# lucaspk512/vrdone

Hardware: AMD Instinct MI355X
Metric: subject-object pairs/sec forward (2048 pairs x 256 frames x 512-d) (higher is better)
Workload: dtype f16x3: f32 products as 3 scaled-f16 MFMA products (~22-bit), f32 accumulate; reference-grade: distance to a float64 run of the reference <= 1.4 x the reference's own float32 error (tests/golden/mask_vrd_f64.npz)

## Files before the change

vrdone_amd/csrc/vrd_gemm_epilogue.h:

```cpp
#pragma once
#include "vrd_common.h"
#include <type_traits>

namespace vrd {

using f32x16 = __attribute__((ext_vector_type(16))) float;
constexpr int STG_PITCH = 64;

typedef float f32x4_t __attribute__((ext_vector_type(4)));
struct acc32q {
    f32x4_t b[2][2];
};
__device__ __forceinline__ void acc_clear(f32x16& a) {
#pragma unroll
    for (int e = 0; e < 16; ++e) a[e] = 0.f;
}
__device__ __forceinline__ void acc_clear(acc32q& a) {
#pragma unroll
    for (int i = 0; i < 2; ++i)
#pragma unroll
        for (int j = 0; j < 2; ++j)
#pragma unroll
            for (int e = 0; e < 4; ++e) a.b[i][j][e] = 0.f;
}
template <typename Fn>
__device__ __forceinline__ void forall32(const f32x16& a, int lane, Fn&& f) {
    const int li = lane & 31, lh = lane >> 5;
#pragma unroll
    for (int e = 0; e < 16; ++e) f((e & 3) + 8 * (e >> 2) + 4 * lh, li, a[e]);
}
template <typename Fn>
__device__ __forceinline__ void forall32(const acc32q& a, int lane, Fn&& f) {
    const int lc = lane & 15, lq = lane >> 4;
#pragma unroll
    for (int bi = 0; bi < 2; ++bi)
#pragma unroll
        for (int bj = 0; bj < 2; ++bj)
#pragma unroll
            for (int j = 0; j < 4; ++j) f(16 * bi + 4 * lq + j, 16 * bj + lc, a.b[bi][bj][j]);
}

__device__ __forceinline__ float epilogue_value(const vrd_gemm_args& p, float v, float mk, float scale, float r1, float rmk,
                                                float r2) {
    if (p.act == VRD_ACT_RELU) v = fmaxf(v, 0.f);
    else if (p.act == VRD_ACT_GELU) v = gelu_erf(v);
    return v * mk * scale + r1 * rmk + r2;
}

struct EpiCols {
    float bias[4], scale[4];
    float alpha;
};
__device__ __forceinline__ float acc_alpha(const vrd_gemm_args& p) {
    if (!(p.split_fmt == VRD_PAIR_F16 && p.w_scale)) return 1.0f;
    const float alpha = uniform_load(p.w_scale);
    return (p.a_scale && p.a_pair_width == 0) ? alpha * F16_ACT_SCALE * uniform_load(p.a_scale + 1) : alpha;
}
__device__ __forceinline__ EpiCols load_epi_cols(const vrd_gemm_args& p, int nw, int lane) {
    EpiCols c;
    c.alpha = acc_alpha(p);
    const int n = nw + (lane & 15) * 4;
#pragma unroll
    for (int j = 0; j < 4; ++j) c.bias[j] = 0.f, c.scale[j] = 1.f;
    if (n + 3 < p.N) {
        if (p.bias) {
            const float4 b = gload4(p.bias + n);
            c.bias[0] = b.x, c.bias[1] = b.y, c.bias[2] = b.z, c.bias[3] = b.w;
        }
        if (p.scale) {
            const float4 b = gload4(p.scale + n);
            c.scale[0] = b.x, c.scale[1] = b.y, c.scale[2] = b.z, c.scale[3] = b.w;
        }
    }
    return c;
}

__device__ __forceinline__ EpiCols load_epi_cols_async(const vrd_gemm_args& p, int nw, int lane) {
    EpiCols c;
    c.alpha = acc_alpha(p);
    const int n = nw + (lane & 15) * 4;
    float4 b = make_float4(0.f, 0.f, 0.f, 0.f), sc = make_float4(1.f, 1.f, 1.f, 1.f);
    if (n + 3 < p.N) {
        if (p.bias) asm volatile("global_load_dwordx4 %0, %1, off" : "=v"(b) : "v"(p.bias + n) : "memory");
        if (p.scale) asm volatile("global_load_dwordx4 %0, %1, off" : "=v"(sc) : "v"(p.scale + n) : "memory");
    }
    c.bias[0] = b.x, c.bias[1] = b.y, c.bias[2] = b.z, c.bias[3] = b.w;
    c.scale[0] = sc.x, c.scale[1] = sc.y, c.scale[2] = sc.z, c.scale[3] = sc.w;
    return c;
}

template <bool ROWIN, int ACT, int SLAB, int ROWS, typename Transposer>
__device__ __forceinline__ void gemm_epilogue_lean_tr(const vrd_gemm_args& p, Transposer&& transpose_into, float* stg, int64_t mw,
                                                      int64_t mw1, int nw, int lane, const EpiCols& cols, unsigned* rflag = nullptr) {
    RangeTrack rt;
    const int64_t hop = mw1 - (mw + 32);
    const int c4 = (lane & 15) * 4, rb0 = lane >> 4;
    const int n = nw + c4;
    const int64_t m_lane = mw + rb0;
    const bool pair = p.c_pair != 0;
    char* const c_lane = reinterpret_cast<char*>(p.C + m_lane * p.ldc) + (pair ? pair_index(n) * 2 : n * 4);
    const float* const r1_lane = (ROWIN && p.res) ? p.res + m_lane * p.ldres + n : nullptr;
    const float* const r2_lane = (ROWIN && p.res2) ? p.res2 + m_lane * p.ldres2 + n : nullptr;
    const unsigned char* const mk_lane = (ROWIN && p.row_mask) ? p.row_mask + m_lane : nullptr;
    const int64_t c_step = p.ldc * 16, r1_step = p.ldres * 4, r2_step = p.ldres2 * 4;
    const int64_t c_hop = hop * p.ldc * 4;
    struct RowIn {
        unsigned char mb[4];
        float4 r1[4], r2[4];
    };
    auto fetch = [&](int pass) {
        RowIn in;
        if (ROWIN) {
            if (p.row_mask) {
#pragma unroll
                for (int j = 0; j < 4; ++j) in.mb[j] = *as_global(mk_lane + pass * 16 + 4 * j + (pass >= 2 ? hop : 0));
            }
            if (p.res) {
#pragma unroll
                for (int j = 0; j < 4; ++j)
                    in.r1[j] = gload4(r1_lane + (pass * 4 + j) * r1_step + (pass >= 2 ? hop * p.ldres : 0));
            }
            if (p.res2) {
#pragma unroll
                for (int j = 0; j < 4; ++j)
                    in.r2[j] = gload4(r2_lane + (pass * 4 + j) * r2_step + (pass >= 2 ? hop * p.ldres2 : 0));
            }
        }
        return in;
    };
    constexpr int NPASS = ROWS / 16;
    RowIn q0 = fetch(0), q1 = fetch(1);
    unsigned rd_addr[4];
    {
        typedef __attribute__((address_space(3))) const float* lds_cf;
#pragma unroll
        for (int j = 0; j < 4; ++j) rd_addr[j] = (unsigned)reinterpret_cast<uintptr_t>((lds_cf)(stg + (rb0 + 4 * j) * STG_PITCH + (c4 ^ (16 * j))));
    }
    transpose_into(stg, SLAB == 64 ? -1 : 0);
#pragma unroll
    for (int pass = 0; pass < NPASS; ++pass) {
        if (SLAB == 32 && pass == 2) transpose_into(stg, 1);
        const RowIn cur = q0;
        q0 = q1;
        if (pass + 2 < NPASS) q1 = fetch(pass + 2);
        float v[4][4];
        float4 tr[4];
        {
            constexpr int PASS_OFF = (SLAB == 64 ? 1 : 0);
            const int poff = (PASS_OFF ? pass : (pass & 1)) * 16 * STG_PITCH * 4;
            asm volatile("ds_read_b128 %0, %4 offset:%8\n\tds_read_b128 %1, %5 offset:%8\n\tds_read_b128 %2, %6 offset:%8\n\tds_read_b128 %3, %7 offset:%8\n\t"
                         "s_waitcnt lgkmcnt(0)"
                         : "=&v"(tr[0]), "=&v"(tr[1]), "=&v"(tr[2]), "=&v"(tr[3])
                         : "v"(rd_addr[0]), "v"(rd_addr[1]), "v"(rd_addr[2]), "v"(rd_addr[3]), "n"(poff)
                         : "memory");
        }
#pragma unroll
        for (int j = 0; j < 4; ++j) {
            const float4 t = tr[j];
            v[j][0] = fmaf(t.x, cols.alpha, cols.bias[0]), v[j][1] = fmaf(t.y, cols.alpha, cols.bias[1]);
            v[j][2] = fmaf(t.z, cols.alpha, cols.bias[2]), v[j][3] = fmaf(t.w, cols.alpha, cols.bias[3]);
        }
        if (ACT == VRD_ACT_GELU) {
#pragma unroll
            for (int j = 0; j < 4; ++j)
#pragma unroll
                for (int c = 0; c < 4; c += 2) {
                    f32x2_t t2;
                    t2.x = v[j][c], t2.y = v[j][c + 1];
                    t2 = gelu_erf2(t2);
                    v[j][c] = t2.x, v[j][c + 1] = t2.y;
                }
        }
        if (ROWIN) {
            float mk[4] = {1.f, 1.f, 1.f, 1.f};
            if (p.row_mask) {
#pragma unroll
                for (int j = 0; j < 4; ++j) mk[j] = (float)cur.mb[j];
            }
            if (p.row_mask || p.scale) {
#pragma unroll
                for (int j = 0; j < 4; ++j)
#pragma unroll
                    for (int c = 0; c < 4; ++c) v[j][c] *= mk[j] * cols.scale[c];
            }
            if (p.res) {
#pragma unroll
                for (int j = 0; j < 4; ++j) {
                    const float rmk = p.res_masked ? mk[j] : 1.f;
                    v[j][0] += cur.r1[j].x * rmk, v[j][1] += cur.r1[j].y * rmk;
                    v[j][2] += cur.r1[j].z * rmk, v[j][3] += cur.r1[j].w * rmk;
                }
            }
            if (p.res2) {
#pragma unroll
                for (int j = 0; j < 4; ++j) {
                    v[j][0] += cur.r2[j].x, v[j][1] += cur.r2[j].y;
                    v[j][2] += cur.r2[j].z, v[j][3] += cur.r2[j].w;
                }
            }
        }
        if (pair) {
            if (p.c_pair == VRD_PAIR_F16) {
#pragma unroll
                for (int j = 0; j < 4; ++j) {
                    char* const rowp = c_lane + (pass * 4 + j) * c_step + (pass >= 2 ? c_hop : 0);
                    f16x4_t h, l;
                    split_n<true>(v[j], h, l, &rt);
                    *as_global(reinterpret_cast<f16x4_t*>(rowp)) = h;
                    *as_global(reinterpret_cast<f16x4_t*>(rowp + 64)) = l;
                }
            } else {
#pragma unroll
                for (int j = 0; j < 4; ++j) {
                    char* const rowp = c_lane + (pass * 4 + j) * c_step + (pass >= 2 ? c_hop : 0);
                    bf16x4_t h, l;
                    split_n<false>(v[j], h, l);
                    *as_global(reinterpret_cast<bf16x4_t*>(rowp)) = h;
                    *as_global(reinterpret_cast<bf16x4_t*>(rowp + 64)) = l;
                }
            }
        } else {
#pragma unroll
            for (int j = 0; j < 4; ++j)
                gstore4(c_lane + (pass * 4 + j) * c_step + (pass >= 2 ? c_hop : 0), make_float4(v[j][0], v[j][1], v[j][2], v[j][3]));
        }
    }
    if (p.c_pair == VRD_PAIR_F16) rt.report(rflag, RANGE_GEMM_OUT);
}

template <bool ROWIN, int ACT, int SLAB = 64>
__device__ __forceinline__ void gemm_epilogue_lean16(const vrd_gemm_args& p, const f32x4_t (&acc)[4][4], float* stg, int64_t mw,
                                                     int64_t mw1, int nw, int lane, const EpiCols& cols, unsigned* rflag = nullptr) {
    const int lc = lane & 15, lq = lane >> 4;
    gemm_epilogue_lean_tr<ROWIN, ACT, SLAB, 64>(
        p,
        [&](float* slab, int half) {
#pragma unroll
            for (int ti = 0; ti < 4; ++ti) {
                if (half >= 0 && (ti >> 1) != half) continue;
                const int r0 = half < 0 ? ti * 16 : (ti & 1) * 16;
#pragma unroll
                for (int tj = 0; tj < 4; ++tj)
#pragma unroll
                    for (int j = 0; j < 4; ++j) slab[(r0 + 4 * lq + j) * STG_PITCH + (tj ^ lq) * 16 + lc] = acc[ti][tj][j];
            }
        },
        stg, mw, mw1, nw, lane, cols, rflag);
}

inline bool gemm_epilogue_lean_ok(const vrd_gemm_args& a) {
    auto al16 = [](const void* q) { return (reinterpret_cast<uintptr_t>(q) & 15u) == 0; };
    return a.M % 64 == 0 && a.N % 64 == 0 && (a.act == VRD_ACT_NONE || a.act == VRD_ACT_GELU) &&
           !(a.act == VRD_ACT_GELU && (a.row_mask || a.scale || a.res || a.res2)) && al16(a.bias) && al16(a.scale);
}

template <bool STAGED, int SLAB_ROWS = 32, typename Acc>
__device__ __forceinline__ void gemm_epilogue(const vrd_gemm_args& p, const Acc (&acc)[2][2], float* smem, int64_t mw,
                                              int nw, int wave, int lane, unsigned* rflag = nullptr, int64_t mw1 = -1) {
    if (mw1 < 0) mw1 = mw + 32;
    auto rowbase = [&](int mi) { return mi ? mw1 : mw; };
    RangeTrack rt;
    constexpr bool SWZ = std::is_same<Acc, acc32q>::value;
    if (STAGED) {
        float* stg = smem + wave * (SLAB_ROWS * STG_PITCH);
        const int c4 = (lane & 15) * 4, rb0 = lane >> 4;
        const int n = nw + c4;
        const bool nfull = n + 3 < p.N;
        const float alpha = acc_alpha(p);
        float bias[4] = {0.f, 0.f, 0.f, 0.f}, scale[4] = {1.f, 1.f, 1.f, 1.f};
        if (nfull && ((reinterpret_cast<uintptr_t>(p.bias) | reinterpret_cast<uintptr_t>(p.scale)) & 15) == 0) {
            if (p.bias) {
                const float4 b = *reinterpret_cast<const float4*>(p.bias + n);
                bias[0] = b.x, bias[1] = b.y, bias[2] = b.z, bias[3] = b.w;
            }
            if (p.scale) {
                const float4 b = *reinterpret_cast<const float4*>(p.scale + n);
                scale[0] = b.x, scale[1] = b.y, scale[2] = b.z, scale[3] = b.w;
            }
        } else {
#pragma unroll
            for (int j = 0; j < 4; ++j)
                if (n + j < p.N) {
                    if (p.bias) bias[j] = p.bias[n + j];
                    if (p.scale) scale[j] = p.scale[n + j];
                }
        }
        const bool row_inputs = p.row_mask || p.res || p.res2;
        const bool ragged = __any(n < p.N && !nfull);
        struct RowIn {
            float mk[4];
            float4 r1[4], r2[4];
        };
        auto fetch = [&](int pass) {
            RowIn in;
#pragma unroll
            for (int j = 0; j < 4; ++j) {
                in.mk[j] = 1.f;
                in.r1[j] = make_float4(0.f, 0.f, 0.f, 0.f);
                in.r2[j] = in.r1[j];
            }
            if (!row_inputs) return in;
            const int64_t mr = rowbase(pass >> 1) + rb0 + (pass & 1) * 16;
            if (!ragged) {
                const int nc = n < p.N ? n : 0;
                unsigned char mb[4];
                int64_t mc[4];
#pragma unroll
                for (int j = 0; j < 4; ++j) mc[j] = (mr + 4 * j < p.M) ? mr + 4 * j : p.M - 1;
                if (p.row_mask) {
#pragma unroll
                    for (int j = 0; j < 4; ++j) mb[j] = p.row_mask[mc[j]];
                }
                if (p.res) {
#pragma unroll
                    for (int j = 0; j < 4; ++j) in.r1[j] = *reinterpret_cast<const float4*>(p.res + mc[j] * p.ldres + nc);
                }
                if (p.res2) {
#pragma unroll
                    for (int j = 0; j < 4; ++j) in.r2[j] = *reinterpret_cast<const float4*>(p.res2 + mc[j] * p.ldres2 + nc);
                }
                if (p.row_mask) {
#pragma unroll
                    for (int j = 0; j < 4; ++j) in.mk[j] = (float)mb[j];
                }
                return in;
            }
#pragma unroll
            for (int j = 0; j < 4; ++j) {
                const int64_t m = mr + 4 * j;
                const bool ok = m < p.M && n < p.N;
                if (p.row_mask && ok) in.mk[j] = (float)p.row_mask[m];
                if (ok && nfull) {
                    if (p.res) in.r1[j] = *reinterpret_cast<const float4*>(p.res + m * p.ldres + n);
                    if (p.res2) in.r2[j] = *reinterpret_cast<const float4*>(p.res2 + m * p.ldres2 + n);
                } else if (ok) {
                    float a1[4] = {0.f, 0.f, 0.f, 0.f}, a2[4] = {0.f, 0.f, 0.f, 0.f};
#pragma unroll
                    for (int c = 0; c < 4; ++c)
                        if (n + c < p.N) {
                            if (p.res) a1[c] = p.res[m * p.ldres + n + c];
                            if (p.res2) a2[c] = p.res2[m * p.ldres2 + n + c];
                        }
                    in.r1[j] = make_float4(a1[0], a1[1], a1[2], a1[3]);
                    in.r2[j] = make_float4(a2[0], a2[1], a2[2], a2[3]);
                }
            }
            return in;
        };
        RowIn cur = fetch(0);
#pragma unroll
        for (int pass = 0; pass < 4; ++pass) {
            const int mi = pass >> 1, h = pass & 1;
            const int slab_row0 = SLAB_ROWS == 64 ? mi * 32 : 0;
            if (SLAB_ROWS == 64 ? pass == 0 : h == 0) {
#pragma unroll
                for (int mt = 0; mt < 2; ++mt) {
                    if (SLAB_ROWS == 64 ? false : mt != mi) continue;
#pragma unroll
                    for (int nj = 0; nj < 2; ++nj)
                        forall32(acc[mt][nj], lane, [&](int r, int c, float x) {
                            stg[((SLAB_ROWS == 64 ? mt * 32 : 0) + r) * STG_PITCH + ((nj * 32 + c) ^ (SWZ ? ((r >> 2) & 3) << 4 : 0))] = x;
                        });
                }
            }
            RowIn nxt = cur;
            if (pass + 1 < 4) nxt = fetch(pass + 1);
            float v[4][4];
#pragma unroll
            for (int j = 0; j < 4; ++j) {
                const float4 t = *reinterpret_cast<const float4*>(stg + (slab_row0 + rb0 + h * 16 + 4 * j) * STG_PITCH + (c4 ^ (SWZ ? 16 * j : 0)));
                v[j][0] = fmaf(t.x, alpha, bias[0]), v[j][1] = fmaf(t.y, alpha, bias[1]);
                v[j][2] = fmaf(t.z, alpha, bias[2]), v[j][3] = fmaf(t.w, alpha, bias[3]);
            }
            if (p.act == VRD_ACT_GELU) {
#pragma unroll
                for (int j = 0; j < 4; ++j)
#pragma unroll
                    for (int c = 0; c < 4; ++c) v[j][c] = gelu_erf(v[j][c]);
            } else if (p.act == VRD_ACT_RELU) {
#pragma unroll
                for (int j = 0; j < 4; ++j)
#pragma unroll
                    for (int c = 0; c < 4; ++c) v[j][c] = fmaxf(v[j][c], 0.f);
            }
#pragma unroll
            for (int j = 0; j < 4; ++j) {
                const float rmk = p.res_masked ? cur.mk[j] : 1.f;
                const float a1[4] = {cur.r1[j].x, cur.r1[j].y, cur.r1[j].z, cur.r1[j].w};
                const float a2[4] = {cur.r2[j].x, cur.r2[j].y, cur.r2[j].z, cur.r2[j].w};
#pragma unroll
                for (int c = 0; c < 4; ++c) v[j][c] = v[j][c] * cur.mk[j] * scale[c] + a1[c] * rmk + a2[c];
            }
#pragma unroll
            for (int j = 0; j < 4; ++j) {
                const int64_t m = rowbase(mi) + rb0 + h * 16 + 4 * j;
                if (m >= p.M || n >= p.N) continue;
                float* crow = p.C + m * p.ldc + n;
                if (p.c_pair) {
                    store_pair4(p.C + m * p.ldc, n, p.N, make_float4(v[j][0], v[j][1], v[j][2], v[j][3]), p.c_pair, &rt);
                } else if (nfull) {
                    *reinterpret_cast<float4*>(crow) = make_float4(v[j][0], v[j][1], v[j][2], v[j][3]);
                } else {
#pragma unroll
                    for (int c = 0; c < 4; ++c)
                        if (n + c < p.N) crow[c] = v[j][c];
                }
            }
            cur = nxt;
        }
        if (p.c_pair == VRD_PAIR_F16) rt.report(rflag, RANGE_GEMM_OUT);
        return;
    }
    const float alpha = acc_alpha(p);
#pragma unroll
    for (int nj = 0; nj < 2; ++nj)
#pragma unroll
        for (int mi = 0; mi < 2; ++mi)
            forall32(acc[mi][nj], lane, [&](int r, int c, float x) {
                const int n = nw + nj * 32 + c;
                const int64_t m = rowbase(mi) + r;
                if (n >= p.N || m >= p.M) return;
                const float bias = p.bias ? p.bias[n] : 0.f;
                const float scale = p.scale ? p.scale[n] : 1.f;
                const float mk = p.row_mask ? (float)p.row_mask[m] : 1.f;
                const float r1 = p.res ? p.res[m * p.ldres + n] : 0.f;
                const float r2 = p.res2 ? p.res2[m * p.ldres2 + n] : 0.f;
                const float v = epilogue_value(p, fmaf(x, alpha, bias), mk, scale, r1, p.res_masked ? mk : 1.f, r2);
                if (p.c_pair) store_pair1(p.C + m * p.ldc, n, p.N, v, p.c_pair, &rt);
                else p.C[m * p.ldc + n] = v;
            });
    if (p.c_pair == VRD_PAIR_F16) rt.report(rflag, RANGE_GEMM_OUT);
}

template <typename Acc>
__device__ __forceinline__ void gemm_epilogue_tile32(const vrd_gemm_args& p, const Acc& acc, int64_t mw, int nw, int lane,
                                                     unsigned* rflag = nullptr) {
    RangeTrack rt;
    const float alpha = acc_alpha(p);
    forall32(acc, lane, [&](int r, int c, float x) {
        const int n = nw + c;
        const int64_t m = mw + r;
        if (n >= p.N || m >= p.M) return;
        const float bias = p.bias ? p.bias[n] : 0.f;
        const float scale = p.scale ? p.scale[n] : 1.f;
        const float mk = p.row_mask ? (float)p.row_mask[m] : 1.f;
        const float r1 = p.res ? p.res[m * p.ldres + n] : 0.f;
        const float r2 = p.res2 ? p.res2[m * p.ldres2 + n] : 0.f;
        const float v = epilogue_value(p, fmaf(x, alpha, bias), mk, scale, r1, p.res_masked ? mk : 1.f, r2);
        if (p.c_pair) store_pair1(p.C + m * p.ldc, n, p.N, v, p.c_pair, &rt);
        else p.C[m * p.ldc + n] = v;
    });
    if (p.c_pair == VRD_PAIR_F16) rt.report(rflag, RANGE_GEMM_OUT);
}

}
```

vrdone_amd/csrc/vrd_gemm_x3_big.hip:

```cpp
#include "vrd_common.h"
#include "vrd_gemm_epilogue.h"
#include <cstdlib>
#include <type_traits>

namespace {

typedef __attribute__((address_space(3))) void* lds_ptr_t;

constexpr int TM = 256, TN = 256;
constexpr int ROWB = 128;
constexpr int A_STAGE = TM * ROWB, W_STAGE = TN * ROWB;
constexpr int NA_STG = 3, NW_STG = 2;
__attribute__((unused)) constexpr int W_RING = NA_STG * A_STAGE;
constexpr size_t BIG_LDS = (size_t)NA_STG * A_STAGE + (size_t)NW_STG * W_STAGE;
__attribute__((unused)) constexpr int PER = 4;
__device__ unsigned long long g_big_skipped_kn;

#ifndef VRD_LAB_STAMP
#define LAB_STAMP(slot)
#define LAB_REAL(slot)
#define LAB_PHASE_DECL
#define LAB_PHASE(i)
#define LAB_PHASE_FLUSH(grp)
#else
#undef LAB_STAMP
#undef LAB_REAL
#undef LAB_PHASE_FLUSH
#define LAB_STAMP(slot)                                                                        \
    do {                                                                                       \
        if (threadIdx.x == 0 && vb < 65536) g_lab[vb * 8 + (slot)] = __builtin_amdgcn_s_memtime(); \
    } while (0)
#define LAB_REAL(slot)                                                                         \
    do {                                                                                       \
        if (threadIdx.x == 0 && vb < 65536) g_lab[vb * 8 + (slot)] = __builtin_amdgcn_s_memrealtime(); \
    } while (0)
#define LAB_PHASE_FLUSH(grp)                                                                   \
    do {                                                                                       \
        if ((threadIdx.x & 255) == 0 && vb < 4096)                                             \
            for (int i_ = 0; i_ < 5; ++i_) g_lab_phase[vb * 16 + (grp) * 8 + i_] = lab_acc[i_]; \
    } while (0)
#endif

__device__ constexpr int swz(int row) { return (row >> 1) & 7; }

struct BigBatch {
    const float* A[3];
    const uint16_t* W_split[3];
    const float* bias[3];
    float* C[3];
    const float* w_scale[3];
};

struct BigKArgs {
    vrd_gemm_args p;
    int tiles_m, tiles_n;
    BigBatch bb;
    int stagger;
    int count;
    unsigned* rflag;
};
typedef const __attribute__((address_space(4))) unsigned* kargs_ptr_t;
template <typename T>
__device__ __forceinline__ T load_karg(kargs_ptr_t base, int byte_off) {
    constexpr int N = (sizeof(T) + 3) / 4;
    unsigned tmp[N];
#pragma unroll
    for (int i = 0; i < N; ++i) tmp[i] = base[byte_off / 4 + i];
    T out;
    __builtin_memcpy(&out, tmp, sizeof(T));
    return out;
}

template <int TAPS, bool PERSIST, bool F16, int WH, int NPROD>
__device__ __forceinline__ void gemm_x3_big_body() {
    static_assert(NPROD == 3 || (NPROD == 1 && F16), "the one-product form exists for the f16 format only");
#if defined(__HIP_DEVICE_COMPILE__)
    constexpr bool LO = NPROD == 3;
    constexpr int KB = LO ? 1 : 2;
    constexpr int NQ = LO ? 12 : 8;
    typedef typename vrd::SplitFmt<F16>::x8 e16x8;
    kargs_ptr_t kp = (kargs_ptr_t)__builtin_amdgcn_kernarg_segment_ptr();
    vrd_gemm_args p;
    int tiles_m, tiles_n, K, nkt, nwg, nblk;
    const int32_t* rb;
    int64_t a_pstride, w_pstride;
    int zsel = PERSIST ? 0 : (int)blockIdx.y;
    auto reload = [&]() __attribute__((always_inline)) {
        if (PERSIST) asm volatile("" : "+s"(kp));
        p = load_karg<vrd_gemm_args>(kp, offsetof(BigKArgs, p));
        tiles_m = load_karg<int>(kp, offsetof(BigKArgs, tiles_m));
        tiles_n = load_karg<int>(kp, offsetof(BigKArgs, tiles_n));
        if (zsel) {
            const BigBatch bb = load_karg<BigBatch>(kp, offsetof(BigKArgs, bb));
            const int z = zsel;
            p.A = z == 1 ? bb.A[0] : z == 2 ? bb.A[1] : bb.A[2];
            p.w_scale = z == 1 ? bb.w_scale[0] : z == 2 ? bb.w_scale[1] : bb.w_scale[2];
            p.W_split = z == 1 ? bb.W_split[0] : z == 2 ? bb.W_split[1] : bb.W_split[2];
            p.bias = z == 1 ? bb.bias[0] : z == 2 ? bb.bias[1] : bb.bias[2];
            p.C = z == 1 ? bb.C[0] : z == 2 ? bb.C[1] : bb.C[2];
        }
        K = p.Cin * TAPS;
        nkt = K / (32 * KB);
        nwg = tiles_m * tiles_n;
        nblk = (int)(p.M >> 5);
        rb = p.row_blocks;
        a_pstride = p.lda * 32, w_pstride = (int64_t)K * 32;
    };
    reload();
    const int stagger = PERSIST ? 0 : load_karg<int>(kp, offsetof(BigKArgs, stagger));
    unsigned* rflag = nullptr;
    if (stagger && blockIdx.y == 0 && blockIdx.x < 256) {
        const int n = ((blockIdx.x >> 3) & 31) * stagger;
        for (int i = 0; i < n; ++i) __builtin_amdgcn_s_sleep(16);
    }
    extern __shared__ __attribute__((aligned(16))) float smem[];
    char* const lds = reinterpret_cast<char*>(smem);
    const int tid = threadIdx.x;
    const int lane = tid & 63;
    const int wave = WH * 4 + (__builtin_amdgcn_readfirstlane(tid >> 6) & 3);
    const int wm = WH, wn = wave & 3;
    auto blk_of = [&](int slot) { return slot < nblk ? (rb ? vrd::uniform_load(rb + slot) : slot) : -1; };
    struct Tile {
        int tm, n0;
        bool contract;
    };
    auto tile_of = [&](int vb_) {
        const int xcd = vb_ & 7, q = nwg >> 3, rem = nwg & 7;
        const int lid = (xcd < rem ? xcd * (q + 1) : rem * (q + 1) + (xcd - rem) * q) + (vb_ >> 3);
        Tile t;
        t.tm = lid / tiles_n;
        t.n0 = (lid - t.tm * tiles_n) * TN;
        t.contract = true;
        if (rb) {
            const int seg_len = p.row_block_seg_len;
            const int seg = (t.tm * 8) / seg_len;
            t.contract = t.tm * 8 < nblk && t.tm * 8 - seg * seg_len < vrd::uniform_load(p.row_blocks_active + seg);
        }
        return t;
    };
    const int rin = lane >> 3, pch = lane & 7;
    const int row0 = wave * PER * 8 + rin;
    const int chunk0 = (pch ^ swz(row0)) * 16;
    unsigned va[2], vw[2];
    auto lane_offsets = [&]() {
        const unsigned a_lane = (unsigned)rin * (unsigned)(p.lda * 4), w_lane = (unsigned)rin * (unsigned)(K * 4);
        if (LO) {
            va[0] = a_lane + chunk0, va[1] = a_lane + (chunk0 ^ 64);
            vw[0] = w_lane + chunk0, vw[1] = w_lane + (chunk0 ^ 64);
        } else {
            const unsigned c0 = chunk0 >> 4, c1 = c0 ^ 4;
            const unsigned s0 = (c0 & 3) * 16 + (c0 >> 2) * 128, s1 = (c1 & 3) * 16 + (c1 >> 2) * 128;
            va[0] = a_lane + s0, va[1] = a_lane + s1;
            vw[0] = w_lane + s0, vw[1] = w_lane + s1;
        }
    };
    lane_offsets();
    struct Src {
        int tseq0, a_in, w_last;
        __amdgpu_buffer_rsrc_t ra, rw;
    };
    auto src_of = [&](const Tile& t) {
        const int my_blk = blk_of(t.tm * 8 + wave);
        const int64_t a_row = (int64_t)(my_blk < 0 ? 0 : my_blk) * 32 + rin;
        Src r;
        r.tseq0 = (TAPS == 3) ? (int)(a_row % p.T) : 0;
        r.a_in = my_blk < 0 ? 0 : PER;
        const int w_in = (p.N - t.n0 - wave * PER * 8 + 7) / 8;
        r.w_last = (w_in > 0 ? (w_in < PER ? w_in : PER) : 1) - 1;
        const int64_t a_row_u = (int64_t)(my_blk < 0 ? 0 : my_blk) * 32 - (TAPS == 3 ? 1 : 0);
        r.ra = __builtin_amdgcn_make_buffer_rsrc(const_cast<float*>(p.A + a_row_u * p.lda), 0, 0x80000000u, 0x00020000);
        r.rw = __builtin_amdgcn_make_buffer_rsrc(
            const_cast<char*>(reinterpret_cast<const char*>(p.W_split) + (int64_t)(t.n0 + (w_in > 0 ? wave * PER * 8 : 0)) * K * 4), 0,
            0x80000000u, 0x00020000);
        return r;
    };
    auto issue_w1 = [&](const Src& c, int gk, int ks, int i) {
        char* const dst = lds + W_RING + (gk % NW_STG) * W_STAGE + wave * PER * 1024;
        __builtin_amdgcn_raw_ptr_buffer_load_lds(c.rw, (lds_ptr_t)(dst + i * 1024), 16, vw[i & 1],
                                                 (i < c.w_last ? i : c.w_last) * (int)w_pstride + ks * 128 * KB, 0, 0);
    };
    auto issue_a1 = [&](const Src& c, int gk, int ks, int i) {
        char* const dst = lds + (gk % NA_STG) * A_STAGE + wave * PER * 1024;
        const int k0 = ks * 32 * KB;
        int tap = 0, ci0 = k0;
        unsigned vo = va[i & 1];
        if (TAPS == 3) {
            tap = (k0 >= p.Cin) + (k0 >= 2 * p.Cin);
            ci0 = k0 - tap * p.Cin;
            int tt = c.tseq0 + 8 * i;
            if (tt >= p.T) tt -= p.T;
            tt += tap - 1;
            if (tt < 0 || tt >= p.T || i >= c.a_in) vo = 0x80000000u;
        }
        __builtin_amdgcn_raw_ptr_buffer_load_lds(c.ra, (lds_ptr_t)(dst + i * 1024), 16, vo,
                                                 i * (int)a_pstride + tap * (int)(p.lda * 4) + ci0 * 4, 0, 0);
    };
    auto issue_w = [&](const Src& c, int gk, int ks) {
#pragma unroll
        for (int i = 0; i < PER; ++i) issue_w1(c, gk, ks, i);
    };
    auto issue_a = [&](const Src& c, int gk, int ks) {
#pragma unroll
        for (int i = 0; i < PER; ++i) issue_a1(c, gk, ks, i);
    };

    bool staged = false;
    bool stored_all = false;
    int g0 = 0;
    const int count = PERSIST ? load_karg<int>(kp, offsetof(BigKArgs, count)) : 1;
    int vq = blockIdx.x, vb = blockIdx.x;
#ifdef VRD_BIG_NOCARRY
    constexpr bool CARRY = false;
#else
    constexpr bool CARRY = true;
#endif
    Tile nt_keep = Tile{0, 0, false};
    Src nx_keep = src_of(nt_keep);
    do {
    if (PERSIST) {
        zsel = (vq >= nwg) + (vq >= 2 * nwg) + (vq >= 3 * nwg);
        vb = vq - zsel * nwg;
        if (vq != (int)blockIdx.x || zsel) reload();
    }
    LAB_STAMP(0);
    LAB_REAL(4);
    const Tile tile = (PERSIST && staged && CARRY) ? nt_keep : tile_of(vb);
    const int tm = tile.tm, n0 = tile.n0;
    const bool contract = tile.contract;
    const Src cur = (PERSIST && staged && CARRY) ? nx_keep : src_of(tile);
    bool next_staged = false;
    Src nx = cur;
    if (PERSIST && contract && vb + (int)gridDim.x < nwg) {
        const Tile nt = tile_of(vb + (int)gridDim.x);
        if (nt.contract) {
            nx = src_of(nt);
            next_staged = true;
            nt_keep = nt;
        }
    }
    nx_keep = nx;
    if (!contract && tid == 0 && tm * 8 < nblk)
        atomicAdd(&g_big_skipped_kn, (unsigned long long)K * (unsigned)(p.N - n0 < TN ? p.N - n0 : TN));

    const int l15 = lane & 15, l4 = lane >> 4;
    int a_hi_off = (wm * 128 + l15) * ROWB + ((l4 ^ swz(l15)) * 16), a_lo_off = a_hi_off ^ 64;
    int w_hi_off = W_RING + (wn * 64 + l15) * ROWB + ((l4 ^ swz(l15)) * 16), w_lo_off = w_hi_off ^ 64;
    asm volatile("" : "+v"(a_hi_off), "+v"(a_lo_off), "+v"(w_hi_off), "+v"(w_lo_off));

    const vrd::EpiCols cols = vrd::load_epi_cols_async(p, n0 + wn * 64, lane);
    vrd::f32x4_t acc[8][4];
    if (!contract) {
        float z;
        asm volatile("v_mov_b32 %0, 0" : "=v"(z));
#pragma unroll
        for (int i = 0; i < 8; ++i)
#pragma unroll
            for (int j = 0; j < 4; ++j)
#pragma unroll
                for (int e = 0; e < 4; ++e) acc[i][j][e] = z;
    }

    struct AF { e16x8 hi, lo; };
    struct WF { e16x8 hi[4], lo[4]; };
    auto load_a = [&](const char* sa, int mi) {
        AF f;
        f.hi = *reinterpret_cast<const e16x8*>(sa + a_hi_off + mi * 16 * ROWB);
        f.lo = *reinterpret_cast<const e16x8*>(sa + a_lo_off + mi * 16 * ROWB);
        return f;
    };
    auto load_w1 = [&](const char* sw, int t, WF& f) {
        f.hi[t] = *reinterpret_cast<const e16x8*>(sw + w_hi_off + t * 16 * ROWB);
        f.lo[t] = *reinterpret_cast<const e16x8*>(sw + w_lo_off + t * 16 * ROWB);
    };
    if (contract) {
    if (!(PERSIST && staged)) {
        issue_a(cur, g0, 0);
        issue_w(cur, g0, 0);
        issue_a(cur, g0 + 1, 1);
        issue_w(cur, g0 + 1, 1);
        LAB_STAMP(1);
        asm volatile("s_waitcnt vmcnt(%0)" ::"n"(2 * PER) : "memory");
    } else {
        issue_w(cur, g0 + 1, 1);
        LAB_STAMP(1);
        if (stored_all) asm volatile("s_waitcnt vmcnt(%0)" ::"n"(2 * PER + 32) : "memory");
        else asm volatile("s_waitcnt vmcnt(%0)" ::"n"(2 * PER) : "memory");
    }
    LAB_STAMP(6);
    __builtin_amdgcn_s_barrier();
    LAB_STAMP(7);
    WF w_cur;
#pragma unroll
    for (int t = 0; t < 4; ++t) load_w1(lds + (g0 % NW_STG) * W_STAGE, t, w_cur);
    AF a_cur = load_a(lds + (g0 % NA_STG) * A_STAGE, 0), a_nxt = a_cur;
    LAB_PHASE_DECL;
    enum { POS_FIRST, POS_STEADY, POS_PEN, POS_LAST };
    auto kstep = [&](int kt, auto pos_c) __attribute__((always_inline)) {
        constexpr int POS = decltype(pos_c)::value;
        auto dma_slot = [&](int kt_open, int d, bool w_ok, bool a_ok) {
            if (d < PER) {
                if (w_ok) issue_w1(cur, g0 + kt_open + 2, kt_open + 2, d);
            } else {
                if (a_ok) issue_a1(cur, g0 + kt_open + 3, kt_open + 3, d - PER);
            }
        };
        auto dma_slot_next = [&](int j_w, int j_a, int d) {
            if (d < PER) issue_w1(nx, g0 + nkt + j_w, j_w, d);
            else issue_a1(nx, g0 + nkt + j_a, j_a, d - PER);
        };
        const char* sa = lds + ((g0 + kt) % NA_STG) * A_STAGE;
        const char* sa1 = lds + ((g0 + kt + 1) % NA_STG) * A_STAGE;
        const char* sw1 = lds + ((g0 + kt + 1) % NW_STG) * W_STAGE;
        constexpr bool last = POS == POS_LAST;
#pragma unroll
        for (int g = 0; g < 8; ++g) {
            if (g == 0) __builtin_amdgcn_s_setprio(3);
            if (g == 2) __builtin_amdgcn_s_setprio(2);
            if (g == 4) __builtin_amdgcn_s_setprio(1);
            if (g == 6) __builtin_amdgcn_s_setprio(0);
            if (g < 7) a_nxt = load_a(sa, g + 1);
            if (g == 7 && !last) a_nxt = load_a(sa1, 0);
            auto dma_of_group = [&]() __attribute__((always_inline)) {
                __builtin_amdgcn_sched_barrier(0);
#ifdef VRD_LAB_NODMA
                if (POS == POS_STEADY) return;
#endif
                if (g < 7) {
                    if (POS == POS_FIRST) {
                        if (g < PER) issue_a1(cur, g0 + 2, 2, g);
                    } else if (POS == POS_STEADY) {
                        dma_slot(kt - 1, g + 1, true, true);
                    } else if (POS == POS_PEN) {
                        if (g + 1 < PER) dma_slot(kt - 1, g + 1, true, false);
                        else if (PERSIST) dma_slot_next(0, 0, g + 1);
                    } else if (POS == POS_LAST && PERSIST) {
                        dma_slot_next(0, 1, g + 1);
                    }
                } else if (!last) {
                    if (POS == POS_PEN && PERSIST) dma_slot_next(0, 0, 0);
                    else dma_slot(kt, 0, POS != POS_PEN, false);
                }
                __builtin_amdgcn_sched_barrier(0);
            };
            constexpr bool blockmajor = !last;
#pragma unroll
            for (int q = 0; q < NQ; ++q) {
                const int pr = LO ? ((blockmajor && g == 7) ? q % 3 : q >> 2) : 0;
                const int kb = LO ? 0 : ((blockmajor && g == 7) ? q & 1 : q >> 2);
                const int t = LO ? ((blockmajor && g == 7) ? q / 3 : q & 3) : ((blockmajor && g == 7) ? q >> 1 : q & 3);
                const bool a_lo = LO ? pr == 0 : kb == 1, w_lo = LO ? pr == 1 : kb == 1;
                const bool chain0 = LO ? pr == 0 : kb == 0, w_done = LO ? pr == 2 : kb == 1;
                const vrd::f32x4_t zero4 = {0.f, 0.f, 0.f, 0.f};
                acc[g][t] = vrd::mfma16(a_lo ? a_cur.lo : a_cur.hi, w_lo ? w_cur.lo[t] : w_cur.hi[t],
                                        (POS == POS_FIRST && chain0) ? zero4 : acc[g][t]);
                if (blockmajor && g == 7 && w_done) load_w1(sw1, t, w_cur);
                if ((q == NQ / 2 - 1 && WH == 0) || (q == NQ - 1 && WH == 1)) dma_of_group();
            }
            a_cur = a_nxt;
            if (g == 6 && !last) {
                asm volatile("s_waitcnt lgkmcnt(0)" ::: "memory");
                LAB_PHASE(3);
                if (POS != POS_PEN || PERSIST) asm volatile("s_waitcnt vmcnt(%0)" ::"n"(PER) : "memory");
                else asm volatile("s_waitcnt vmcnt(0)" ::: "memory");
                LAB_PHASE(0);
                __builtin_amdgcn_sched_barrier(0);
                __builtin_amdgcn_s_barrier();
                __builtin_amdgcn_sched_barrier(0);
                LAB_PHASE(1);
            }
        }
    };
    kstep(0, std::integral_constant<int, POS_FIRST>{});
    for (int kt = 1; kt + 2 < nkt; ++kt) kstep(kt, std::integral_constant<int, POS_STEADY>{});
    kstep(nkt - 2, std::integral_constant<int, POS_PEN>{});
    kstep(nkt - 1, std::integral_constant<int, POS_LAST>{});
    LAB_PHASE_FLUSH(WH);
    __builtin_amdgcn_s_setprio(0);
    }
#ifdef VRD_LAB_STAMP
    asm volatile("" ::"v"(acc[0][0][0]));
#endif
    if (!contract) asm volatile("s_waitcnt vmcnt(0)" ::: "memory");
    asm volatile("s_waitcnt lgkmcnt(0)" ::: "memory");
    __builtin_amdgcn_s_barrier();
    LAB_STAMP(2);
    rflag = load_karg<unsigned*>(kp, offsetof(BigKArgs, rflag));
    if (PERSIST) {
        reload();
        staged = next_staged;
    }
    const int slab_a = ((g0 + nkt + 2) % NA_STG) * A_STAGE, slab_w = W_RING + ((g0 + nkt + 1) % NW_STG) * W_STAGE;
    float* const stg = PERSIST ? smem + ((wave < 4 ? slab_a : slab_w - 4 * (32 * vrd::STG_PITCH * 4)) + wave * (32 * vrd::STG_PITCH * 4)) / 4
                               : smem + wave * (64 * vrd::STG_PITCH);
    bool all_stored = true;
    constexpr int SLAB = PERSIST ? 32 : 64;
    int lane_e = lane;
    asm volatile("" : "+v"(lane_e));
#pragma unroll
    for (int hm = 0; hm < 2; ++hm) {
        const int slot = tm * 8 + wm * 4 + hm * 2;
        const int blk_a = blk_of(slot), blk_b = blk_of(slot + 1);
        const int nw = n0 + wn * 64;
        if (blk_a < 0 || nw >= p.N) {
            all_stored = false;
            continue;
        }
        const int64_t mw = (int64_t)blk_a * 32, mw1 = (int64_t)blk_b * 32;
        const bool rowin = !PERSIST && (p.row_mask || p.scale || p.res || p.res2);
        vrd::f32x4_t part[4][4];
#pragma unroll
        for (int i = 0; i < 4; ++i)
#pragma unroll
            for (int j = 0; j < 4; ++j) part[i][j] = acc[4 * hm + i][j];
        if (rowin) vrd::gemm_epilogue_lean16<true, VRD_ACT_NONE, SLAB>(p, part, stg, mw, mw1, nw, lane_e, cols, rflag);
        else if (p.act == VRD_ACT_GELU) vrd::gemm_epilogue_lean16<false, VRD_ACT_GELU, SLAB>(p, part, stg, mw, mw1, nw, lane_e, cols, rflag);
        else vrd::gemm_epilogue_lean16<false, VRD_ACT_NONE, SLAB>(p, part, stg, mw, mw1, nw, lane_e, cols, rflag);
    }
    LAB_STAMP(3);
    LAB_REAL(5);
    if (PERSIST) {
        asm volatile("s_waitcnt lgkmcnt(0)" ::: "memory");
        __builtin_amdgcn_s_barrier();
    }
    stored_all = all_stored;
    g0 = (g0 + nkt) % 6;
    vq += (int)gridDim.x;
    } while (PERSIST && vq < nwg * count);
    if (PERSIST) asm volatile("s_waitcnt vmcnt(0)" ::: "memory");
#endif
}

template <int TAPS, bool PERSIST, bool F16 = false, int NPROD = 3>
__global__ __launch_bounds__(512) void gemm_x3_big_kernel(BigKArgs ka_unused_) {
    if (__builtin_amdgcn_readfirstlane(threadIdx.x >> 8)) gemm_x3_big_body<TAPS, PERSIST, F16, 1, NPROD>();
    else gemm_x3_big_body<TAPS, PERSIST, F16, 0, NPROD>();
}

}

namespace vrd {

template <int TAPS, bool PERSIST, bool F16 = false, int NPROD = 3>
static int launch_big_one(const vrd_gemm_args& a, hipStream_t s, const BigBatch& bb = BigBatch{}, int count = 1) {
    auto kern = gemm_x3_big_kernel<TAPS, PERSIST, F16, NPROD>;
    if (int rc = reserve_lds(reinterpret_cast<const void*>(kern), BIG_LDS, "vrd_gemm(bf16x3 256x256)")) return rc;
    const int tiles_m = (int)((a.M + TM - 1) / TM), tiles_n = (a.N + TN - 1) / TN;
    const int nwg = tiles_m * tiles_n;
    static const int stagger = [] { const char* e = getenv("VRD_BIG_STAGGER"); return e ? atoi(e) : 2; }();
    const int n_cu = PERSIST ? device_cu_count() : 0;
    BigKArgs ka;
    ka.p = a, ka.tiles_m = tiles_m, ka.tiles_n = tiles_n, ka.bb = bb, ka.stagger = (PERSIST || nwg < 512) ? 0 : stagger;
    ka.rflag = a.c_pair == VRD_PAIR_F16 ? range_flag() : nullptr;
    ka.count = count;
    if (PERSIST) hipLaunchKernelGGL(kern, dim3(nwg * count < n_cu ? nwg * count : n_cu), dim3(512), BIG_LDS, s, ka);
    else hipLaunchKernelGGL(kern, dim3(nwg, count), dim3(512), BIG_LDS, s, ka);
    return 0;
}

static bool big_persist(const vrd_gemm_args& a) {
    static const int persist = [] { const char* e = getenv("VRD_BIG_PERSIST"); return e ? atoi(e) : 1; }();
    return persist && a.taps == 1 && a.Cin >= 96 && !(a.row_mask || a.scale || a.res || a.res2);
}

static int launch_big_any(const vrd_gemm_args& a, hipStream_t s, const BigBatch& bb, int count) {
    const bool f16 = a.split_fmt == VRD_PAIR_F16;
    if (f16 && a.products == 1) {
        if (big_persist(a)) return launch_big_one<1, true, true, 1>(a, s, bb, count);
        return a.taps == 1 ? launch_big_one<1, false, true, 1>(a, s, bb, count) : launch_big_one<3, false, true, 1>(a, s, bb, count);
    }
    if (big_persist(a)) return f16 ? launch_big_one<1, true, true>(a, s, bb, count) : launch_big_one<1, true, false>(a, s, bb, count);
    if (f16) return a.taps == 1 ? launch_big_one<1, false, true>(a, s, bb, count) : launch_big_one<3, false, true>(a, s, bb, count);
    return a.taps == 1 ? launch_big_one<1, false, false>(a, s, bb, count) : launch_big_one<3, false, false>(a, s, bb, count);
}

int launch_gemm_x3_big_batch(const vrd_gemm_args* a, int count, hipStream_t s) {
    BigBatch bb{};
    for (int i = 1; i < count; ++i) {
        bb.A[i - 1] = a[i].A;
        bb.W_split[i - 1] = a[i].W_split;
        bb.bias[i - 1] = a[i].bias;
        bb.C[i - 1] = a[i].C;
        bb.w_scale[i - 1] = a[i].w_scale;
    }
    return launch_big_any(a[0], s, bb, count);
}

double take_big_skipped_flops() {
    unsigned long long v = 0, zero = 0;
    if (hipMemcpyFromSymbol(&v, HIP_SYMBOL(g_big_skipped_kn), sizeof(v)) != hipSuccess) return 0.0;
    (void)hipMemcpyToSymbol(HIP_SYMBOL(g_big_skipped_kn), &zero, sizeof(zero));
    return 2.0 * TM * (double)v;
}

int launch_gemm_x3_big(const vrd_gemm_args& a, hipStream_t s) { return launch_big_any(a, s, BigBatch{}, 1); }

}
```

Before: 15680.

## Overlap persistent-tile epilogue with the next tile's first k-step MFMAs

In the persistent 3-product path, the epilogue of the current tile (LDS drain, bias/alpha/GELU, split and global store) is now interleaved group by group with the first k-step of the next tile, through a new POS_OVL k-step and a LeanBlock16 helper. Accumulator and fragment state move outside the tile loop so the next tile can continue from the carried first step. The goal is to hide the epilogue store and LDS round-trip latency behind MFMA work instead of leaving the matrix units idle between tiles. In exchange the code needs more live registers, uses hand-tuned vmcnt waits that depend on the DMA count, and adds complexity in reusing the LDS ring slots, all of which could hurt occupancy or correctness.

```diff
diff --git a/vrdone_amd/csrc/vrd_gemm_epilogue.h b/vrdone_amd/csrc/vrd_gemm_epilogue.h
--- a/vrdone_amd/csrc/vrd_gemm_epilogue.h
+++ b/vrdone_amd/csrc/vrd_gemm_epilogue.h
@@ -248,6 +248,79 @@
         stg, mw, mw1, nw, lane, cols, rflag);
 }
 
+struct LeanBlock16 {
+    float* wr;
+    unsigned rd[4];
+    int lq;
+    RangeTrack rt;
+    __device__ __forceinline__ LeanBlock16(float* slab, int lane) : lq(lane >> 4) {
+        typedef __attribute__((address_space(3))) const float* lds_cf;
+        const int c4 = (lane & 15) * 4;
+        wr = slab + 4 * lq * STG_PITCH + (lane & 15);
+#pragma unroll
+        for (int j = 0; j < 4; ++j) rd[j] = (unsigned)reinterpret_cast<uintptr_t>((lds_cf)(slab + (lq + 4 * j) * STG_PITCH + (c4 ^ (16 * j))));
+    }
+    __device__ __forceinline__ void drain(const f32x4_t (&a)[4]) const {
+#pragma unroll
+        for (int tj = 0; tj < 4; ++tj)
+#pragma unroll
+            for (int j = 0; j < 4; ++j) wr[j * STG_PITCH + (tj ^ lq) * 16] = a[tj][j];
+    }
+    __device__ __forceinline__ void read(float4 (&tr)[4]) const {
+        asm volatile("ds_read_b128 %0, %4\n\tds_read_b128 %1, %5\n\tds_read_b128 %2, %6\n\tds_read_b128 %3, %7\n\t"
+                     "s_waitcnt lgkmcnt(0)"
+                     : "=&v"(tr[0]), "=&v"(tr[1]), "=&v"(tr[2]), "=&v"(tr[3])
+                     : "v"(rd[0]), "v"(rd[1]), "v"(rd[2]), "v"(rd[3])
+                     : "memory");
+    }
+    __device__ __forceinline__ void finish(const vrd_gemm_args& p, const float4 (&tr)[4], char* c_lane, const EpiCols& cols) {
+        const int64_t c_step = p.ldc * 16;
+        float v[4][4];
+#pragma unroll
+        for (int j = 0; j < 4; ++j) {
+            const float4 t = tr[j];
+            v[j][0] = fmaf(t.x, cols.alpha, cols.bias[0]), v[j][1] = fmaf(t.y, cols.alpha, cols.bias[1]);
+            v[j][2] = fmaf(t.z, cols.alpha, cols.bias[2]), v[j][3] = fmaf(t.w, cols.alpha, cols.bias[3]);
+        }
+        if (p.act == VRD_ACT_GELU) {
+#pragma unroll
+            for (int j = 0; j < 4; ++j)
+#pragma unroll
+                for (int c = 0; c < 4; c += 2) {
+                    f32x2_t t2;
+                    t2.x = v[j][c], t2.y = v[j][c + 1];
+                    t2 = gelu_erf2(t2);
+                    v[j][c] = t2.x, v[j][c + 1] = t2.y;
+                }
+        }
+        if (p.c_pair == VRD_PAIR_F16) {
+#pragma unroll
+            for (int j = 0; j < 4; ++j) {
+                char* const rowp = c_lane + j * c_step;
+                f16x4_t h, l;
+                split_n<true>(v[j], h, l, &rt);
+                *as_global(reinterpret_cast<f16x4_t*>(rowp)) = h;
+                *as_global(reinterpret_cast<f16x4_t*>(rowp + 64)) = l;
+            }
+        } else if (p.c_pair) {
+#pragma unroll
+            for (int j = 0; j < 4; ++j) {
+                char* const rowp = c_lane + j * c_step;
+                bf16x4_t h, l;
+                split_n<false>(v[j], h, l);
+                *as_global(reinterpret_cast<bf16x4_t*>(rowp)) = h;
+                *as_global(reinterpret_cast<bf16x4_t*>(rowp + 64)) = l;
+            }
+        } else {
+#pragma unroll
+            for (int j = 0; j < 4; ++j) gstore4(c_lane + j * c_step, make_float4(v[j][0], v[j][1], v[j][2], v[j][3]));
+        }
+    }
+    __device__ __forceinline__ void report(const vrd_gemm_args& p, unsigned* rflag) const {
+        if (p.c_pair == VRD_PAIR_F16) rt.report(rflag, RANGE_GEMM_OUT);
+    }
+};
+
 inline bool gemm_epilogue_lean_ok(const vrd_gemm_args& a) {
     auto al16 = [](const void* q) { return (reinterpret_cast<uintptr_t>(q) & 15u) == 0; };
     return a.M % 64 == 0 && a.N % 64 == 0 && (a.act == VRD_ACT_NONE || a.act == VRD_ACT_GELU) &&
diff --git a/vrdone_amd/csrc/vrd_gemm_x3_big.hip b/vrdone_amd/csrc/vrd_gemm_x3_big.hip
--- a/vrdone_amd/csrc/vrd_gemm_x3_big.hip
+++ b/vrdone_amd/csrc/vrd_gemm_x3_big.hip
@@ -40,6 +40,17 @@
             for (int i_ = 0; i_ < 5; ++i_) g_lab_phase[vb * 16 + (grp) * 8 + i_] = lab_acc[i_]; \
     } while (0)
 #endif
+
+template <typename D, typename F, typename W>
+struct OvHooks {
+    D drain;
+    F finish;
+    W wait_stage1;
+};
+template <typename D, typename F, typename W>
+__device__ __forceinline__ OvHooks<D, F, W> make_ov_hooks(D d, F f, W w) {
+    return OvHooks<D, F, W>{d, f, w};
+}
 
 __device__ constexpr int swz(int row) { return (row >> 1) & 7; }
 
@@ -216,6 +227,13 @@
 #endif
     Tile nt_keep = Tile{0, 0, false};
     Src nx_keep = src_of(nt_keep);
+    constexpr bool OVL = PERSIST && NPROD == 3;
+    struct AF { e16x8 hi, lo; };
+    struct WF { e16x8 hi[4], lo[4]; };
+    vrd::f32x4_t acc[8][4];
+    WF w_cur;
+    AF a_cur, a_nxt;
+    bool carried = false;
     do {
     if (PERSIST) {
         zsel = (vq >= nwg) + (vq >= 2 * nwg) + (vq >= 3 * nwg);
@@ -248,7 +266,6 @@
     asm volatile("" : "+v"(a_hi_off), "+v"(a_lo_off), "+v"(w_hi_off), "+v"(w_lo_off));
 
     const vrd::EpiCols cols = vrd::load_epi_cols_async(p, n0 + wn * 64, lane);
-    vrd::f32x4_t acc[8][4];
     if (!contract) {
         float z;
         asm volatile("v_mov_b32 %0, 0" : "=v"(z));
@@ -260,8 +277,6 @@
                 for (int e = 0; e < 4; ++e) acc[i][j][e] = z;
     }
 
-    struct AF { e16x8 hi, lo; };
-    struct WF { e16x8 hi[4], lo[4]; };
     auto load_a = [&](const char* sa, int mi) {
         AF f;
         f.hi = *reinterpret_cast<const e16x8*>(sa + a_hi_off + mi * 16 * ROWB);
@@ -272,7 +287,99 @@
         f.hi[t] = *reinterpret_cast<const e16x8*>(sw + w_hi_off + t * 16 * ROWB);
         f.lo[t] = *reinterpret_cast<const e16x8*>(sw + w_lo_off + t * 16 * ROWB);
     };
+    LAB_PHASE_DECL;
+    enum { POS_FIRST, POS_STEADY, POS_PEN, POS_LAST, POS_OVL };
+    auto kstep = [&](int kt, auto pos_c, auto&& ov) __attribute__((always_inline)) {
+        constexpr int POS = decltype(pos_c)::value;
+        constexpr bool FIRST = POS == POS_FIRST || POS == POS_OVL;
+        const int gb = POS == POS_OVL ? g0 + nkt : g0;
+        auto dma_slot = [&](int kt_open, int d, bool w_ok, bool a_ok) {
+            if (d < PER) {
+                if (w_ok) issue_w1(cur, g0 + kt_open + 2, kt_open + 2, d);
+            } else {
+                if (a_ok) issue_a1(cur, g0 + kt_open + 3, kt_open + 3, d - PER);
+            }
+        };
+        auto dma_slot_next = [&](int j_w, int j_a, int d) {
+            if (d < PER) issue_w1(nx, g0 + nkt + j_w, j_w, d);
+            else issue_a1(nx, g0 + nkt + j_a, j_a, d - PER);
+        };
+        const char* sa = lds + ((gb + kt) % NA_STG) * A_STAGE;
+        const char* sa1 = lds + ((gb + kt + 1) % NA_STG) * A_STAGE;
+        const char* sw1 = lds + ((gb + kt + 1) % NW_STG) * W_STAGE;
+        constexpr bool last = POS == POS_LAST;
+#pragma unroll
+        for (int g = 0; g < 8; ++g) {
+            if (POS != POS_OVL) {
+                if (g == 0) __builtin_amdgcn_s_setprio(3);
+                if (g == 2) __builtin_amdgcn_s_setprio(2);
+                if (g == 4) __builtin_amdgcn_s_setprio(1);
+                if (g == 6) __builtin_amdgcn_s_setprio(0);
+            }
+            if constexpr (POS == POS_OVL) {
+                ov.drain(g);
+                if (WH == 1) ov.finish(g);
+            }
+            if (g < 7) a_nxt = load_a(sa, g + 1);
+            if (g == 7 && !last) a_nxt = load_a(sa1, 0);
+            auto dma_of_group = [&]() __attribute__((always_inline)) {
+                __builtin_amdgcn_sched_barrier(0);
+#ifdef VRD_LAB_NODMA
+                if (POS == POS_STEADY) return;
+#endif
+                if (g < 7) {
+                    if (POS == POS_OVL) {
+                    } else if (POS == POS_FIRST) {
+                        if (g < PER) issue_a1(cur, g0 + 2, 2, g);
+                    } else if (POS == POS_STEADY) {
+                        dma_slot(kt - 1, g + 1, true, true);
+                    } else if (POS == POS_PEN) {
+                        if (g + 1 < PER) dma_slot(kt - 1, g + 1, true, false);
+                        else if (PERSIST) dma_slot_next(0, 0, g + 1);
+                    } else if (POS == POS_LAST && PERSIST) {
+                        dma_slot_next(0, 1, g + 1);
+                    }
+                } else if (!last) {
+                    if (POS == POS_PEN && PERSIST) dma_slot_next(0, 0, 0);
+                    else if (POS == POS_OVL) issue_w1(nx, gb + 2, 2, 0);
+                    else dma_slot(kt, 0, POS != POS_PEN, false);
+                }
+                __builtin_amdgcn_sched_barrier(0);
+            };
+            constexpr bool blockmajor = !last;
+#pragma unroll
+            for (int q = 0; q < NQ; ++q) {
+                const int pr = LO ? ((blockmajor && g == 7) ? q % 3 : q >> 2) : 0;
+                const int kb = LO ? 0 : ((blockmajor && g == 7) ? q & 1 : q >> 2);
+                const int t = LO ? ((blockmajor && g == 7) ? q / 3 : q & 3) : ((blockmajor && g == 7) ? q >> 1 : q & 3);
+                const bool a_lo = LO ? pr == 0 : kb == 1, w_lo = LO ? pr == 1 : kb == 1;
+                const bool chain0 = LO ? pr == 0 : kb == 0, w_done = LO ? pr == 2 : kb == 1;
+                const vrd::f32x4_t zero4 = {0.f, 0.f, 0.f, 0.f};
+                acc[g][t] = vrd::mfma16(a_lo ? a_cur.lo : a_cur.hi, w_lo ? w_cur.lo[t] : w_cur.hi[t],
+                                        (FIRST && chain0) ? zero4 : acc[g][t]);
+                if (blockmajor && g == 7 && w_done) load_w1(sw1, t, w_cur);
+                if ((q == NQ / 2 - 1 && WH == 0) || (q == NQ - 1 && WH == 1)) dma_of_group();
+            }
+            a_cur = a_nxt;
+            if constexpr (POS == POS_OVL) {
+                if (WH == 0) ov.finish(g);
+            }
+            if (g == 6 && !last) {
+                asm volatile("s_waitcnt lgkmcnt(0)" ::: "memory");
+                LAB_PHASE(3);
+                if constexpr (POS == POS_OVL) ov.wait_stage1();
+                else if (POS != POS_PEN || PERSIST) asm volatile("s_waitcnt vmcnt(%0)" ::"n"(PER) : "memory");
+                else asm volatile("s_waitcnt vmcnt(0)" ::: "memory");
+                LAB_PHASE(0);
+                __builtin_amdgcn_sched_barrier(0);
+                __builtin_amdgcn_s_barrier();
+                __builtin_amdgcn_sched_barrier(0);
+                LAB_PHASE(1);
+            }
+        }
+    };
     if (contract) {
+    if (!(OVL && carried)) {
     if (!(PERSIST && staged)) {
         issue_a(cur, g0, 0);
         issue_w(cur, g0, 0);
@@ -289,91 +396,18 @@
     LAB_STAMP(6);
     __builtin_amdgcn_s_barrier();
     LAB_STAMP(7);
-    WF w_cur;
 #pragma unroll
     for (int t = 0; t < 4; ++t) load_w1(lds + (g0 % NW_STG) * W_STAGE, t, w_cur);
-    AF a_cur = load_a(lds + (g0 % NA_STG) * A_STAGE, 0), a_nxt = a_cur;
-    LAB_PHASE_DECL;
-    enum { POS_FIRST, POS_STEADY, POS_PEN, POS_LAST };
-    auto kstep = [&](int kt, auto pos_c) __attribute__((always_inline)) {
-        constexpr int POS = decltype(pos_c)::value;
-        auto dma_slot = [&](int kt_open, int d, bool w_ok, bool a_ok) {
-            if (d < PER) {
-                if (w_ok) issue_w1(cur, g0 + kt_open + 2, kt_open + 2, d);
-            } else {
-                if (a_ok) issue_a1(cur, g0 + kt_open + 3, kt_open + 3, d - PER);
-            }
-        };
-        auto dma_slot_next = [&](int j_w, int j_a, int d) {
-            if (d < PER) issue_w1(nx, g0 + nkt + j_w, j_w, d);
-            else issue_a1(nx, g0 + nkt + j_a, j_a, d - PER);
-        };
-        const char* sa = lds + ((g0 + kt) % NA_STG) * A_STAGE;
-        const char* sa1 = lds + ((g0 + kt + 1) % NA_STG) * A_STAGE;
-        const char* sw1 = lds + ((g0 + kt + 1) % NW_STG) * W_STAGE;
-        constexpr bool last = POS == POS_LAST;
-#pragma unroll
-        for (int g = 0; g < 8; ++g) {
-            if (g == 0) __builtin_amdgcn_s_setprio(3);
-            if (g == 2) __builtin_amdgcn_s_setprio(2);
-            if (g == 4) __builtin_amdgcn_s_setprio(1);
-            if (g == 6) __builtin_amdgcn_s_setprio(0);
-            if (g < 7) a_nxt = load_a(sa, g + 1);
-            if (g == 7 && !last) a_nxt = load_a(sa1, 0);
-            auto dma_of_group = [&]() __attribute__((always_inline)) {
-                __builtin_amdgcn_sched_barrier(0);
-#ifdef VRD_LAB_NODMA
-                if (POS == POS_STEADY) return;
-#endif
-                if (g < 7) {
-                    if (POS == POS_FIRST) {
-                        if (g < PER) issue_a1(cur, g0 + 2, 2, g);
-                    } else if (POS == POS_STEADY) {
-                        dma_slot(kt - 1, g + 1, true, true);
-                    } else if (POS == POS_PEN) {
-                        if (g + 1 < PER) dma_slot(kt - 1, g + 1, true, false);
-                        else if (PERSIST) dma_slot_next(0, 0, g + 1);
-                    } else if (POS == POS_LAST && PERSIST) {
-                        dma_slot_next(0, 1, g + 1);
-                    }
-                } else if (!last) {
-                    if (POS == POS_PEN && PERSIST) dma_slot_next(0, 0, 0);
-                    else dma_slot(kt, 0, POS != POS_PEN, false);
-                }
-                __builtin_amdgcn_sched_barrier(0);
-            };
-            constexpr bool blockmajor = !last;
-#pragma unroll
-            for (int q = 0; q < NQ; ++q) {
-                const int pr = LO ? ((blockmajor && g == 7) ? q % 3 : q >> 2) : 0;
-                const int kb = LO ? 0 : ((blockmajor && g == 7) ? q & 1 : q >> 2);
-                const int t = LO ? ((blockmajor && g == 7) ? q / 3 : q & 3) : ((blockmajor && g == 7) ? q >> 1 : q & 3);
-                const bool a_lo = LO ? pr == 0 : kb == 1, w_lo = LO ? pr == 1 : kb == 1;
-                const bool chain0 = LO ? pr == 0 : kb == 0, w_done = LO ? pr == 2 : kb == 1;
-                const vrd::f32x4_t zero4 = {0.f, 0.f, 0.f, 0.f};
-                acc[g][t] = vrd::mfma16(a_lo ? a_cur.lo : a_cur.hi, w_lo ? w_cur.lo[t] : w_cur.hi[t],
-                                        (POS == POS_FIRST && chain0) ? zero4 : acc[g][t]);
-                if (blockmajor && g == 7 && w_done) load_w1(sw1, t, w_cur);
-                if ((q == NQ / 2 - 1 && WH == 0) || (q == NQ - 1 && WH == 1)) dma_of_group();
-            }
-            a_cur = a_nxt;
-            if (g == 6 && !last) {
-                asm volatile("s_waitcnt lgkmcnt(0)" ::: "memory");
-                LAB_PHASE(3);
-                if (POS != POS_PEN || PERSIST) asm volatile("s_waitcnt vmcnt(%0)" ::"n"(PER) : "memory");
-                else asm volatile("s_waitcnt vmcnt(0)" ::: "memory");
-                LAB_PHASE(0);
-                __builtin_amdgcn_sched_barrier(0);
-                __builtin_amdgcn_s_barrier();
-                __builtin_amdgcn_sched_barrier(0);
-                LAB_PHASE(1);
-            }
-        }
-    };
-    kstep(0, std::integral_constant<int, POS_FIRST>{});
-    for (int kt = 1; kt + 2 < nkt; ++kt) kstep(kt, std::integral_constant<int, POS_STEADY>{});
-    kstep(nkt - 2, std::integral_constant<int, POS_PEN>{});
-    kstep(nkt - 1, std::integral_constant<int, POS_LAST>{});
+    a_cur = load_a(lds + (g0 % NA_STG) * A_STAGE, 0), a_nxt = a_cur;
+    kstep(0, std::integral_constant<int, POS_FIRST>{}, 0);
+    } else {
+        LAB_STAMP(1);
+        LAB_STAMP(6);
+        LAB_STAMP(7);
+    }
+    for (int kt = 1; kt + 2 < nkt; ++kt) kstep(kt, std::integral_constant<int, POS_STEADY>{}, 0);
+    kstep(nkt - 2, std::integral_constant<int, POS_PEN>{}, 0);
+    kstep(nkt - 1, std::integral_constant<int, POS_LAST>{}, 0);
     LAB_PHASE_FLUSH(WH);
     __builtin_amdgcn_s_setprio(0);
     }
@@ -389,6 +423,45 @@
         reload();
         staged = next_staged;
     }
+    bool ovl = false;
+    if (OVL) ovl = next_staged && n0 + TN <= p.N && tm * 8 + 8 <= nblk;
+    if (OVL && ovl) {
+        const int gb = g0 + nkt;
+        issue_w(nx, gb + 1, 1);
+        asm volatile("s_waitcnt vmcnt(%0)" ::"n"(2 * PER) : "memory");
+        __builtin_amdgcn_s_barrier();
+#pragma unroll
+        for (int t = 0; t < 4; ++t) load_w1(lds + (gb % NW_STG) * W_STAGE, t, w_cur);
+        a_cur = load_a(lds + (gb % NA_STG) * A_STAGE, 0), a_nxt = a_cur;
+        int lane_e = lane;
+        asm volatile("" : "+v"(lane_e));
+        vrd::LeanBlock16 lb(smem + (((gb + 2) % NA_STG) * A_STAGE + wave * (16 * vrd::STG_PITCH * 4)) / 4, lane_e);
+        static_assert(16 * vrd::STG_PITCH * 4 == PER * 1024, "a wave's 16-row slab is where its own pieces of a stage land");
+        const int n_lane = n0 + wn * 64 + (lane_e & 15) * 4;
+        const int col_b = p.c_pair ? vrd::pair_index(n_lane) * 2 : n_lane * 4;
+        auto ov = make_ov_hooks(
+            [&](int g) __attribute__((always_inline)) { lb.drain(acc[g]); },
+            [&](int g) __attribute__((always_inline)) {
+                const int blk = blk_of(tm * 8 + wm * 4 + (g >> 1));
+                char* const c_lane = reinterpret_cast<char*>(p.C + ((int64_t)blk * 32 + (g & 1) * 16 + lb.lq) * p.ldc) + col_b;
+                float4 tr[4];
+                lb.read(tr);
+                if (g == 7) {
+                    issue_a(nx, gb + 2, 2);
+                }
+                lb.finish(p, tr, c_lane, cols);
+            },
+            [&]() __attribute__((always_inline)) {
+                if (p.c_pair) asm volatile("s_waitcnt vmcnt(%0)" ::"n"(7 * 8) : "memory");
+                else asm volatile("s_waitcnt vmcnt(%0)" ::"n"(7 * 4) : "memory");
+            });
+        kstep(0, std::integral_constant<int, POS_OVL>{}, ov);
+        lb.report(p, rflag);
+        LAB_STAMP(3);
+        LAB_REAL(5);
+        carried = true;
+    } else {
+    carried = false;
     const int slab_a = ((g0 + nkt + 2) % NA_STG) * A_STAGE, slab_w = W_RING + ((g0 + nkt + 1) % NW_STG) * W_STAGE;
     float* const stg = PERSIST ? smem + ((wave < 4 ? slab_a : slab_w - 4 * (32 * vrd::STG_PITCH * 4)) + wave * (32 * vrd::STG_PITCH * 4)) / 4
                                : smem + wave * (64 * vrd::STG_PITCH);
@@ -423,6 +496,7 @@
         __builtin_amdgcn_s_barrier();
     }
     stored_all = all_stored;
+    }
     g0 = (g0 + nkt) % 6;
     vq += (int)gridDim.x;
     } while (PERSIST && vq < nwg * count);
```

Result: no change. 15690 (median of 4 runs) (+0.1%).
